# hguo/ftk

Hardware: AMD Instinct MI355X
Metric: space-time simplices/sec (higher is better)
Workload: dtype int64

## Files before the change

ftk_amd/csrc/mask_kernels.hip:

```cpp
#include <atomic>
#include "internal.hpp"
#include "mask_plan.hpp"
#include "sweep_device.hpp"
#include "series_device.hpp"

namespace ftkx {

__device__ inline void red_commit(u64 *red, double mn, double mx, unsigned slot)
{
  for (int o = 32; o > 0; o >>= 1) { mn = fmin(mn, __shfl_down(mn, o)); mx = fmax(mx, __shfl_down(mx, o)); }
  if ((threadIdx.x & 63) == 0) {
    atomicMin(&red[2 * (slot & 63u)], (u64)__double_as_longlong(mn));
    atomicMax(&red[2 * (slot & 63u) + 1], (u64)__double_as_longlong(mx));
  }
}

template <int ND>
__global__ __launch_bounds__(kThreads) void mask_kernel(const Mesh m, const MaskJob *__restrict__ jobs)
{
  const MaskJob job = jobs[blockIdx.y];
  const int P = m.mask_pitch, DH = m.ext_sz[1], DD = (ND == 3) ? m.ext_sz[2] : 1;
  const size_t n = (size_t)P * DH * DD;
  double red_mn = DBL_MAX, red_mx = 0.0;
  for (size_t idx = (size_t)blockIdx.x * kThreads + threadIdx.x; idx < n; idx += (size_t)gridDim.x * kThreads) {
// ... 540 lines not shown
            if (cmask & 0x00ffu) { take(dx0 * fx2); take(dy0 * fy2); }
            if (cmask & 0xff00u) { take(dx1 * fx2); take(dy1 * fy2); }
          }
        }
        if (per_vertex_rule) {
          asm volatile("" ::: "memory");
          const double m0 = max_abs2(dx0 * fx2, dy0 * fy2), m1 = max_abs2(dx1 * fx2, dy1 * fy2);
          bits = (m0 >= tbig ? 0u : (bits & 0x00ffu)) | (m1 >= tbig ? 0u : (bits & 0xff00u));
        }
      } else {
      shift_in_signs<ND>(a0, a1, dx0, dx1, dy0, dy1, dz0, dz1, tneg, tpos);
      if (ND == 2) { a0 = ((a0 & 0xcu) << 1) | (a0 & 3u); a1 = ((a1 & 0xcu) << 1) | (a1 & 3u); }
      bits = guard_and_reduce<ND>(a0, a1, dx0, dx1, dy0, dy1, dz0, dz1, u_int && rok, cmask, per_vertex_rule, tbig, ND == 3 ? 0.5 : 1.0, acc0, acc1, red_mn);
      }
      const unsigned keep = u_int ? xkeep : 0u;
      const unsigned neut = u_dom ? xneutral : 0x3f3fu;
      bits = (bits & keep) | neut;
      if (block4) { bw[r] = rok ? bits : 0x3f3fu; return; }
      bool word_uniform = false;
      if (have_u) {
        int q = (int)((bits & (bits >> 8)) & 0x3fu);
        q &= __builtin_amdgcn_update_dpp(q, q, 0xb1 , 0xf, 0xf, false);
        q &= __builtin_amdgcn_update_dpp(q, q, 0x4e , 0xf, 0xf, false);
        if (rok && u_lane) __builtin_amdgcn_raw_buffer_store_b8((unsigned char)q, rU, ucol, uplane + (unsigned)m.u_pitch * (unsigned)r, 0);
        word_uniform = q != 0;
      }
      if (rok && store_ok && !word_uniform)
        __builtin_amdgcn_raw_buffer_store_b16((unsigned short)bits, rM, mcol, mplane + (unsigned)P * (unsigned)r, 0);
    });
    if constexpr (ND == 2 && RY % 4 == 0 && !REDUCE) if (block4) {
      static_for<RY / 4>([&](auto bc) {
        constexpr int b = decltype(bc)::value;
        const unsigned all = (bw[4 * b] & bw[4 * b + 1]) & (bw[4 * b + 2] & bw[4 * b + 3]);
        int q = (int)((all & (all >> 8)) & 0x3fu);
        q &= __builtin_amdgcn_update_dpp(q, q, 0xb1 , 0xf, 0xf, false);
        q &= __builtin_amdgcn_update_dpp(q, q, 0x4e , 0xf, 0xf, false);
        const bool first_ok = ((row_ok >> (4 * b)) & 1) && k < z1;
        if (first_ok && u_lane) __builtin_amdgcn_raw_buffer_store_b8((unsigned char)q, rU, ucol, (unsigned)m.u_pitch * ((unsigned)(j0 / 4 + b) + (unsigned)((DH + 3) / 4) * (unsigned)k), 0);
        if (q == 0 && store_ok) {
#pragma unroll
          for (int r = 4 * b; r < 4 * b + 4; r ++)
            if (((row_ok >> r) & 1) && k < z1) __builtin_amdgcn_raw_buffer_store_b16((unsigned short)bw[r], rM, mcol, mplane + (unsigned)P * (unsigned)r, 0);
        }
      });
    }
  };

  v2d B[NB][RY + 2];
  double X[NB];
  for (int b = 0; b < NB; b ++) X[b] = 0.0;
  load_plane(B[0], X[0], z0 - 1);
  load_plane(B[1], X[1], z0);
  if (ND == 3) { for (int b = 2; b < 2 + PD; b ++) load_plane(B[b], X[b], z0 + b - 1 < z1 ? z0 + b - 1 : z1); }
  else for (int b = 2; b < NB; b ++) for (int r = 0; r < RY + 2; r ++) B[b][r] = B[1][r];
  for (int k = z0; k < z1; k += NB) {
#pragma unroll
    for (int i = 0; i < NB; i ++)
      step(B[i], B[(i + 1) % NB], B[(i + 2) % NB], B[(i + 2 + PD) % NB], X[(i + 1) % NB], X[(i + 2 + PD) % NB], k + i);
  }
  const unsigned slot = blockIdx.x + blockIdx.y * 7u + blockIdx.z * 13u + (unsigned)wv;
  if constexpr (REDUCE) red_commit(job.red, red_mn, red_mx, slot);
  else if (job.red) {
    const double h = (ND == 3) ? 0.5 : 1.0;
    double mx = fmax((cmask & 0x00ffu) ? acc0 : 0.0, (cmask & 0xff00u) ? acc1 : 0.0) * h;
    if constexpr (LEAN) {
      const double mxx = fmax((cmask & 0x00ffu) ? acc0 : 0.0, (cmask & 0xff00u) ? acc1 : 0.0) * fx2;
      const double mxy = fmax((cmask & 0x00ffu) ? accy0 : 0.0, (cmask & 0xff00u) ? accy1 : 0.0) * fy2;
      mx = max_plain(mxx, mxy);
    }
    red_commit(job.red, red_mn < job.threshold ? red_mn : DBL_MAX, mx, slot);
  }
}

template <int RY>
__global__ __launch_bounds__(256) void mask_rows2_kernel(const Mesh m, const MaskJob *__restrict__ jobs, int groups, int swizzle)
{
  static_assert(RY == 8, "two 8 x 4 blocks per group; the edge register holds 2 RY <= 16 values");
  const int DW = m.ext_sz[0], DH = m.ext_sz[1], P = m.mask_pitch;
  unsigned bx, by, bz;
  remap_block(swizzle, bx, by, bz);
  const MaskJob job = jobs[bz];
  const int lane = threadIdx.x & 63;
  const int wv = __builtin_amdgcn_readfirstlane((int)(threadIdx.x >> 6));
  const int wpb = blockDim.x >> 6;
  const int i0 = (int)bx * 128 + 2 * lane;
  const int jbase = ((int)by * wpb + wv) * RY * groups;
  if (jbase >= DH) return;
  const int jend = jbase + RY * groups < DH ? jbase + RY * groups : DH;
  const unsigned sy = (unsigned)DW * 8u;
  const __amdgpu_buffer_rsrc_t rS = __builtin_amdgcn_make_buffer_rsrc((void *)job.S, 0, (int)(sy * (unsigned)DH), 0x00020000);
  const __amdgpu_buffer_rsrc_t rM = __builtin_amdgcn_make_buffer_rsrc((void *)job.M, 0, (int)((unsigned)P * (unsigned)DH), 0x00020000);
  const __amdgpu_buffer_rsrc_t rU = __builtin_amdgcn_make_buffer_rsrc((void *)job.U, 0, (int)((unsigned)m.u_pitch * (unsigned)DH), 0x00020000);
  const bool have_u = job.U != nullptr;
  const bool block4 = have_u && m.u_rows == 4;
  const double thr = job.threshold;
  const int ic = i0 < DW ? i0 : DW - 2;
  const unsigned cb = (unsigned)ic * 8u;
  const int t0c = (int)bx * 128;
  const int xr = lane < RY ? lane : (lane >= 64 - RY ? lane - (64 - RY) : -1);
  const unsigned xcol8 = (unsigned)(lane < RY ? (t0c > 0 ? t0c - 1 : 0) : (t0c + 128 < DW ? t0c + 128 : DW - 1)) * 8u;
  unsigned xkeep = 0, xneutral = 0;
  for (int c = 0; c < 2; c ++) {
    const int i = i0 + c;
    const bool x_dom = i < DW && i + m.ext_st[0] >= m.dom_lb[0] && i + m.ext_st[0] <= m.dom_ub[0];
    xkeep |= 0x3fu << (8 * c);
    if (!x_dom) xneutral |= 0x3fu << (8 * c);
  }
  const bool in_row = i0 < DW;
  const unsigned mcol = (unsigned)i0, ucol = (unsigned)(i0 >> 3);
  const bool u_lane = (lane & 3) == 0 && in_row;
  double red_mn = DBL_MAX;
  double acc0 = 0.0, acc1 = 0.0, accy0 = 0.0, accy1 = 0.0;
  const unsigned cmask = in_row ? (xkeep & 0x0303u) : 0u;
  const double tbig = job.big;
  const bool per_vertex_rule = job.big < HUGE_VAL;
  const double fx2 = (double)(DW - 1), fy2 = (double)(DH - 1);
  const double tpx = job.tx > 0.0 ? job.tx : exact_threshold(thr, fx2), tpy = job.ty > 0.0 ? job.ty : exact_threshold(thr, fy2);

  struct Rows { unsigned roff[RY + 2]; unsigned row_dom, row_ok, xoff, cbv; int j0; };
  auto setup = [&](Rows &R, int j0) {
    R.j0 = j0;
    const bool live = j0 < jend;
    R.row_dom = 0; R.row_ok = 0;
    for (int r = 0; r < RY + 2; r ++) {
      const int j = j0 + r - 1;
      R.roff[r] = sy * (unsigned)clampi(j, 0, DH - 1);
      if (r >= 1 && r <= RY) {
        if (j < jend) R.row_ok |= 1u << (r - 1);
        if (j + m.ext_st[1] >= m.dom_lb[1] && j + m.ext_st[1] <= m.dom_ub[1]) R.row_dom |= 1u << (r - 1);
      }
    }
    R.cbv = live ? cb : 0xfffffff0u;
    R.xoff = (live && xr >= 0) ? sy * (unsigned)clampi(j0 + xr, 0, DH - 1) + xcol8 : 0xfffffff0u;
  };
  auto load = [&](v2d (&B)[RY + 2], double &X, const Rows &R) {
    for (int r = 0; r < RY + 2; r ++) B[r] = __builtin_bit_cast(v2d, __builtin_amdgcn_raw_buffer_load_b128(rS, R.cbv, R.roff[r], 0));
    X = __builtin_bit_cast(double, __builtin_amdgcn_raw_buffer_load_b64(rS, R.xoff, 0, 0));
  };
  auto step = [&](const v2d (&CU)[RY + 2], const double XC, const Rows &R) {
    const unsigned mplane = (unsigned)P * (unsigned)R.j0, uplane = (unsigned)m.u_pitch * (unsigned)R.j0;
    unsigned bw[RY];
    static_for<RY>([&](auto rc) {
      constexpr int r = decltype(rc)::value;
      const v2d c = CU[r + 1];
      const double xe = edge_for_row<r, RY>(XC);
      const double xm = dpp_lower_or(c.y, xe);
      double xp = dpp_upper_or(c.x, xe);
      if (i0 + 1 == DW - 1) xp = c.y;
      const double dx0 = c.y - xm, dx1 = xp - c.x;
      const double dy0 = CU[r + 2].x - CU[r].x, dy1 = CU[r + 2].y - CU[r].y;
      const bool rok = (R.row_ok >> r) & 1, u_dom = (R.row_dom >> r) & 1;
      unsigned a0 = 0, a1 = 0;
      shift_in_signs2(a0, a1, dx0, dx1, dy0, dy1, -tpx, tpx, -tpy, tpy);
      unsigned bits = a0 | (a1 << 8);
      if (rok) {
        acc0 = max_with_abs(acc0, dx0); acc1 = max_with_abs(acc1, dx1);
        accy0 = max_with_abs(accy0, dy0); accy1 = max_with_abs(accy1, dy1);
        const unsigned u = bits | (bits >> 3);
        if (__builtin_amdgcn_ballot_w64((~u & cmask) != 0u)) {
          auto take = [&](double g) { const double a = fabs(g); red_mn = fmin(red_mn, a == 0.0 ? DBL_MAX : a); };
          if (cmask & 0x00ffu) { take(dx0 * fx2); take(dy0 * fy2); }
          if (cmask & 0xff00u) { take(dx1 * fx2); take(dy1 * fy2); }
        }
      }
      if (per_vertex_rule) {
        asm volatile("" ::: "memory");
        const double m0 = max_abs2(dx0 * fx2, dy0 * fy2), m1 = max_abs2(dx1 * fx2, dy1 * fy2);
        bits = (m0 >= tbig ? 0u : (bits & 0x00ffu)) | (m1 >= tbig ? 0u : (bits & 0xff00u));
      }
      const unsigned neut = u_dom ? xneutral : 0x3f3fu;
      bits = (bits & xkeep) | neut;
      if (block4) { bw[r] = rok ? bits : 0x3f3fu; return; }
      bool word_uniform = false;
      if (have_u) {
        int q = (int)((bits & (bits >> 8)) & 0x3fu);
        q &= __builtin_amdgcn_update_dpp(q, q, 0xb1 , 0xf, 0xf, false);
        q &= __builtin_amdgcn_update_dpp(q, q, 0x4e , 0xf, 0xf, false);
        if (rok && u_lane) __builtin_amdgcn_raw_buffer_store_b8((unsigned char)q, rU, ucol, uplane + (unsigned)m.u_pitch * (unsigned)r, 0);
        word_uniform = q != 0;
      }
      if (rok && in_row && !word_uniform) __builtin_amdgcn_raw_buffer_store_b16((unsigned short)bits, rM, mcol, mplane + (unsigned)P * (unsigned)r, 0);
    });
    if (block4) {
      static_for<RY / 4>([&](auto bc) {
        constexpr int b = decltype(bc)::value;
        const unsigned all = (bw[4 * b] & bw[4 * b + 1]) & (bw[4 * b + 2] & bw[4 * b + 3]);
        int q = (int)((all & (all >> 8)) & 0x3fu);
        q &= __builtin_amdgcn_update_dpp(q, q, 0xb1 , 0xf, 0xf, false);
        q &= __builtin_amdgcn_update_dpp(q, q, 0x4e , 0xf, 0xf, false);
        const bool first_ok = (R.row_ok >> (4 * b)) & 1;
        if (first_ok && u_lane) __builtin_amdgcn_raw_buffer_store_b8((unsigned char)q, rU, ucol, (unsigned)m.u_pitch * (unsigned)(R.j0 / 4 + b), 0);
        if (q == 0 && in_row) {
#pragma unroll
          for (int r = 4 * b; r < 4 * b + 4; r ++)
            if ((R.row_ok >> r) & 1) __builtin_amdgcn_raw_buffer_store_b16((unsigned short)bw[r], rM, mcol, mplane + (unsigned)P * (unsigned)r, 0);
        }
      });
    }
  };

  Rows Ra, Rb;
  v2d A[RY + 2], B[RY + 2];
  double XA, XB;
  setup(Ra, jbase);
  load(A, XA, Ra);
  for (int g = 0; g < groups; g += 2) {
    setup(Rb, jbase + (g + 1) * RY);
    load(B, XB, Rb);
    step(A, XA, Ra);
    setup(Ra, jbase + (g + 2) * RY);
    load(A, XA, Ra);
    if (g + 1 < groups) step(B, XB, Rb);
  }
  if (job.red) {
    const double mxx = fmax((cmask & 0x00ffu) ? acc0 : 0.0, (cmask & 0xff00u) ? acc1 : 0.0) * fx2;
    const double mxy = fmax((cmask & 0x00ffu) ? accy0 : 0.0, (cmask & 0xff00u) ? accy1 : 0.0) * fy2;
    red_commit(job.red, red_mn < job.threshold ? red_mn : DBL_MAX, max_plain(mxx, mxy), blockIdx.x + blockIdx.y * 7u + blockIdx.z * 13u + (unsigned)wv);
  }
}

template <int R> __device__ inline void pack_pair_and(unsigned &T, unsigned bits)
{
  if constexpr (R == 0) asm("v_and_b32_sdwa %0, %1, %1 dst_sel:BYTE_0 dst_unused:UNUSED_PAD src0_sel:BYTE_0 src1_sel:BYTE_1" : "=v"(T) : "v"(bits));
  else if constexpr (R == 1) asm("v_and_b32_sdwa %0, %1, %1 dst_sel:BYTE_1 dst_unused:UNUSED_PRESERVE src0_sel:BYTE_0 src1_sel:BYTE_1" : "+v"(T) : "v"(bits));
  else if constexpr (R == 2) asm("v_and_b32_sdwa %0, %1, %1 dst_sel:BYTE_2 dst_unused:UNUSED_PRESERVE src0_sel:BYTE_0 src1_sel:BYTE_1" : "+v"(T) : "v"(bits));
  else asm("v_and_b32_sdwa %0, %1, %1 dst_sel:BYTE_3 dst_unused:UNUSED_PRESERVE src0_sel:BYTE_0 src1_sel:BYTE_1" : "+v"(T) : "v"(bits));
}
__device__ inline void quad_and(unsigned &T)
{
  asm("s_nop 1\n\t"
      "v_and_b32_dpp %0, %0, %0 quad_perm:[1,0,3,2] row_mask:0xf bank_mask:0xf\n\t"
      "s_nop 1\n\t"
      "v_and_b32_dpp %0, %0, %0 quad_perm:[2,3,0,1] row_mask:0xf bank_mask:0xf"
      : "+v"(T));
}
__device__ inline void row_quads_or(unsigned &x)
{
  asm("s_nop 1\n\t"
      "v_or_b32_dpp %0, %0, %0 row_ror:4 row_mask:0xf bank_mask:0xf\n\t"
      "s_nop 1\n\t"
      "v_or_b32_dpp %0, %0, %0 row_ror:8 row_mask:0xf bank_mask:0xf"
      : "+v"(x));
}
__device__ inline unsigned select_lanes(unsigned a, unsigned b, unsigned long long mask)
{
  unsigned r;
  asm("v_cndmask_b32_e64 %0, %1, %2, %3" : "=v"(r) : "v"(a), "v"(b), "s"(mask));
  return r;
}
template <int R> __device__ inline void byte_nonzero(unsigned long long &mask, unsigned T, unsigned zero)
{
  if constexpr (R == 0) asm volatile("v_cmp_ne_u32_sdwa %0, %1, %2 src0_sel:BYTE_0 src1_sel:DWORD" : "=s"(mask) : "v"(T), "v"(zero));
  else if constexpr (R == 1) asm volatile("v_cmp_ne_u32_sdwa %0, %1, %2 src0_sel:BYTE_1 src1_sel:DWORD" : "=s"(mask) : "v"(T), "v"(zero));
  else if constexpr (R == 2) asm volatile("v_cmp_ne_u32_sdwa %0, %1, %2 src0_sel:BYTE_2 src1_sel:DWORD" : "=s"(mask) : "v"(T), "v"(zero));
  else asm volatile("v_cmp_ne_u32_sdwa %0, %1, %2 src0_sel:BYTE_3 src1_sel:DWORD" : "=s"(mask) : "v"(T), "v"(zero));
}
__device__ inline unsigned out_of_range_where(unsigned off, unsigned long long mask)
{
  unsigned r;
  asm volatile("v_cndmask_b32_e64 %0, %1, -16, %2" : "=v"(r) : "v"(off), "s"(mask));
  return r;
}
template <int I> __device__ inline void lds_read128(v2d &d, unsigned a) { asm volatile("ds_read_b128 %0, %1 offset:%2" : "=v"(d) : "v"(a), "n"(I * 1024)); }
template <int I> __device__ inline void lds_read64(double &d, unsigned a) { asm volatile("ds_read_b64 %0, %1 offset:%2" : "=v"(d) : "v"(a), "n"(I)); }
__device__ inline void lds_tie(v2d &d) { asm volatile("" : "+v"(d)); }
__device__ inline void lds_tie(double &d) { asm volatile("" : "+v"(d)); }
template <int N, int... I> __device__ inline void lds_rows(v2d (&B)[N], unsigned a, std::integer_sequence<int, I...>) { (lds_read128<I>(B[I], a), ...); }
template <int N, int... I> __device__ inline void lds_tie_rows(v2d (&B)[N], std::integer_sequence<int, I...>) { (lds_tie(B[I]), ...); }
template <int RIGHT, int N, int... I> __device__ inline void lds_edges(double (&XL)[N], double (&XR)[N], unsigned a, std::integer_sequence<int, I...>)
{
  (lds_read64<8 * I>(XL[I], a), ...);
  (lds_read64<RIGHT + 8 * I>(XR[I], a), ...);
}
template <int N, int... I> __device__ inline void lds_tie_edges(double (&XL)[N], double (&XR)[N], std::integer_sequence<int, I...>) { ((lds_tie(XL[I]), lds_tie(XR[I])), ...); }

template <int NS, int RY, int S>
__device__ inline void wait_plane_landed(int s)
{
  static_assert((NS - 1) * RY + NS * S < 64 && NS <= 4, "vmcnt is a 6-bit counter; four early steps are spelled out");
#define FTKX_WAIT_VM(N) __builtin_amdgcn_s_waitcnt(((N) & 15) | (7 << 4) | (15 << 8) | (((N) >> 4) << 14))
  if (s >= NS) FTKX_WAIT_VM((NS - 1) * RY + NS * S);
  else if (s == 1) FTKX_WAIT_VM((NS - 1) * RY + S);
  else if (s == 2) FTKX_WAIT_VM((NS - 1) * RY + 2 * S);
  else if (s == 3) FTKX_WAIT_VM((NS - 1) * RY + 3 * S);
  else FTKX_WAIT_VM((NS - 1) * RY);
#undef FTKX_WAIT_VM
}


template <int NS, int CY, int RY, bool TWOB>
__device__ __forceinline__ void march6_body(const Mesh &m, const MaskJob *__restrict__ jobs, int swizzle, int njobs, const ZPlan &plan)
{
#if defined(__HIP_DEVICE_COMPILE__)
  constexpr int ROWS = RY * CY, TROWS = ROWS + 2, NE = NS + 1;
  constexpr bool EDGE2 = ROWS > 16;
  static_assert(ROWS <= 32 && CY >= (EDGE2 ? 4 : 3), "the odd jobs (two halo rows, edge values) go to different wavefronts");
  constexpr unsigned ROWB = 1024u, SLOT = TROWS * ROWB, EDGEB = EDGE2 ? 512u : 256u, ERIGHT = EDGE2 ? 256u : 128u, ERING = NS * SLOT;
  constexpr int DEPTH = TWOB ? NS : NS - 1;
  static_assert(DEPTH >= 1, "at least one plane on its way");
  extern __shared__ __attribute__((aligned(16))) char lds[];
  const int DW = m.ext_sz[0], DH = m.ext_sz[1], DD = m.ext_sz[2], P = m.mask_pitch;
  unsigned bx, by, bz;
  remap_block(swizzle, bx, by, bz);
  const unsigned nj = (unsigned)(njobs < 0 ? -njobs : njobs);
  const unsigned piece = njobs < 0 ? bz % plan.npieces : bz / nj;
  const MaskJob job = jobs[njobs < 0 ? bz / plan.npieces : bz - piece * nj];
  const int z0 = (int)plan.z0[piece];
  const int z1 = z0 + (int)plan.len[piece];
  const int lane = threadIdx.x & 63;
  const int wv = __builtin_amdgcn_readfirstlane((int)(threadIdx.x >> 6));
  const int jb = (int)by * ROWS, t0c = (int)bx * 128;
  if (jb >= DH) return;
  const unsigned sy = (unsigned)DW * 8u, sz = (unsigned)DW * (unsigned)DH * 8u;
  const __amdgpu_buffer_rsrc_t rS = __builtin_amdgcn_make_buffer_rsrc((void *)job.S, 0, (int)(sz * (unsigned)DD), 0x00020000);
  const int nsteps = ((z1 - z0 + 2) / 3) * 3;
  auto slot_of = [&](int q) -> unsigned { return (unsigned)(((q - (z0 - 1)) % NS + NS) % NS) * SLOT; };
  auto edge_of = [&](int q) -> unsigned { return ERING + (unsigned)(((q - (z0 - 1)) % NE + NE) % NE) * EDGEB; };

  const int ip = t0c + 2 * lane;
  const unsigned cb = (unsigned)(ip < DW ? ip : DW - 2) * 8u;
  unsigned eoff = 0xfffffff0u;
  if (wv == 1 || (EDGE2 && wv == 2)) {
    const int e = lane >> 1, row = EDGE2 ? e : (e & 15);
    const bool left = EDGE2 ? wv == 1 : e < 16;
    if (row < ROWS) {
      const int col = left ? (t0c > 0 ? t0c - 1 : 0) : (t0c + 128 < DW ? t0c + 128 : DW - 1);
      eoff = sy * (unsigned)clampi(jb + row, 0, DH - 1) + (unsigned)col * 8u + 4u * (unsigned)(lane & 1);
    }
  }
  unsigned roff[RY];
  for (int r = 0; r < RY; r ++) roff[r] = sy * (unsigned)clampi(jb + wv * RY + r, 0, DH - 1);
  const int xt = wv == 0 ? 0 : TROWS - 1;
  const unsigned xoff = sy * (unsigned)clampi(jb + xt - 1, 0, DH - 1);
  auto issue = [&](int q) {
    const unsigned zo = sz * (unsigned)clampi(q, 0, DD - 1);
    const unsigned base = slot_of(q);
    for (int r = 0; r < RY; r ++) {
      __attribute__((address_space(3))) void *dst = (__attribute__((address_space(3))) void *)(lds + base + (unsigned)(1 + wv * RY + r) * ROWB);
      __builtin_amdgcn_raw_ptr_buffer_load_lds(rS, dst, 16, cb, zo + roff[r], 0, 0);
    }
    if (wv == 0 || wv == CY - 1) {
      __attribute__((address_space(3))) void *dst = (__attribute__((address_space(3))) void *)(lds + base + (unsigned)xt * ROWB);
      __builtin_amdgcn_raw_ptr_buffer_load_lds(rS, dst, 16, cb, zo + xoff, 0, 0);
    } else if (wv == 1 || (EDGE2 && wv == 2)) {
      __attribute__((address_space(3))) void *edst = (__attribute__((address_space(3))) void *)(lds + edge_of(q) + ((EDGE2 && wv == 2) ? ERIGHT : 0u));
      __builtin_amdgcn_raw_ptr_buffer_load_lds(rS, edst, 4, eoff, zo, 0, 0);
    }
  };
#define FTKX_WAIT_VM(N) __builtin_amdgcn_s_waitcnt(((N) & 15) | (7 << 4) | (15 << 8) | (((N) >> 4) << 14))

  const int wy = wv;
  const int i0 = t0c + 2 * lane;
  const __amdgpu_buffer_rsrc_t rM = __builtin_amdgcn_make_buffer_rsrc((void *)job.M, 0, (int)((unsigned)P * (unsigned)DH * (unsigned)DD), 0x00020000);
  const __amdgpu_buffer_rsrc_t rU = __builtin_amdgcn_make_buffer_rsrc((void *)job.U, 0, job.U ? (int)((unsigned)m.u_pitch * (unsigned)DH * (unsigned)DD) : 0, 0x00020000);
  const double thr = job.threshold;
  const double tpos = 2.0 * thr, tneg = -tpos;
  const int j0 = jb + wy * RY;
  unsigned xkeep = 0, xneutral = 0;
  for (int c = 0; c < 2; c ++) {
    const int i = i0 + c;
    const bool x_dom = i < DW && i + m.ext_st[0] >= m.dom_lb[0] && i + m.ext_st[0] <= m.dom_ub[0];
    const bool x_int = i >= 1 && i < DW - 1;
    if (x_int) xkeep |= 0x3fu << (8 * c);
    if (!x_dom) xneutral |= 0x3fu << (8 * c);
  }
  unsigned row_dom = 0, row_int = 0, row_ok = 0;
  for (int r = 0; r < RY; r ++) {
    const int j = j0 + r;
    if (j < DH) row_ok |= 1u << r;
    if (j + m.ext_st[1] >= m.dom_lb[1] && j + m.ext_st[1] <= m.dom_ub[1]) row_dom |= 1u << r;
    if (j >= 1 && j < DH - 1) row_int |= 1u << r;
  }
  const bool in_row = i0 < DW;
  constexpr unsigned OOB = 0xfffffff0u;
  const bool have_u = job.U != nullptr;
  const unsigned mcol = in_row ? (unsigned)i0 : OOB;
  const unsigned ucol = ((lane & 3) == 0 && in_row && have_u) ? (unsigned)(i0 >> 3) : OOB;
  double acc0 = 0.0, acc1 = 0.0, red_mn = DBL_MAX;
  const unsigned cmask = in_row ? (xkeep & 0x0707u) : 0u;
  const double tbig = 2.0 * job.big;
  const bool per_vertex_rule = job.big < HUGE_VAL;
  const unsigned lds0 = (unsigned)(__UINTPTR_TYPE__)(__attribute__((address_space(3))) char *)lds;
  const unsigned lrow = lds0 + (unsigned)(wy * RY) * ROWB + (unsigned)(lane * 16);
  const unsigned eown = lds0 + (unsigned)(wy * RY) * 8u;
  unsigned uoff[RY], moff[RY];
  for (int r = 0; r < RY; r ++) {
    const bool rok = (row_ok >> r) & 1;
    uoff[r] = (rok && ucol != OOB) ? ucol + (unsigned)m.u_pitch * (unsigned)r : OOB;
    moff[r] = (rok && in_row) ? mcol + (unsigned)P * (unsigned)r : OOB;
  }
  const bool wave_interior = (row_ok & row_int & row_dom) == (1u << RY) - 1u;
  const bool batched = RY == 4 && have_u;
  const bool block4 = batched && m.u_rows == 4;
  const bool block16 = batched && CY == 4 && m.u_rows == 16;
  const bool blk = block4 || block16;
  const unsigned a_l = ((unsigned)lane >> 2) & 3u, r_l = (unsigned)lane & 3u, g_l = (unsigned)lane >> 4;
  const unsigned urows = (unsigned)((DH + m.u_rows - 1) / m.u_rows);
  const unsigned uplane_stride = (unsigned)m.u_pitch * urows;
  const unsigned uo4 = (blk ? ((block4 || wy == 0) && r_l == 0 && (row_ok & 1u)) : ((row_ok >> r_l) & 1u)) ? a_l * uplane_stride + (blk ? 0u : r_l * (unsigned)m.u_pitch) + (unsigned)(t0c >> 3) + 4u * g_l : OOB;
  const unsigned psel = (0x0c0c0c0cu & ~(0xffu << (8u * a_l))) | (r_l << (8u * a_l));
  unsigned uacc = 0u;
  const unsigned vzero = 0u;
  const unsigned xch = lds0 + ERING + (unsigned)NE * EDGEB + (unsigned)(lane >> 2) * 4u;
  unsigned t_prev = 0u;
  int k_prev = 0;
  bool pend = false;
  auto finish_prev = [&](unsigned g4) {
    unsigned t = g4 & (g4 >> 16);
    t &= t >> 8;
    const unsigned G = t & 0xffu;
    const unsigned uplane_prev = (unsigned)m.u_pitch * ((unsigned)(j0 / m.u_rows) + urows * (unsigned)k_prev);
    if (wy == 0) {
      const int j = (k_prev - z0) & 3;
      unsigned c = G << (8u * a_l);
      row_quads_or(c);
      uacc = select_lanes(uacc, c, 0x000f000f000f000full << (4 * j));
      if (j == 3 || k_prev == z1 - 1) {
        const unsigned off = j == 3 ? uo4 : (a_l <= (unsigned)j ? uo4 : OOB);
        __builtin_amdgcn_raw_buffer_store_b32(uacc, rU, off, uplane_prev - (unsigned)j * uplane_stride, 0);
      }
    }
    const bool need = G == 0u && t_prev != 0u;
    if (__builtin_amdgcn_ballot_w64(need)) {
      asm volatile("" ::: "memory");
      const unsigned v = t_prev | (t_prev << 8);
      const unsigned mp = (unsigned)P * ((unsigned)j0 + (unsigned)DH * (unsigned)k_prev);
      static_for<RY>([&](auto rc) { constexpr int r = decltype(rc)::value; __builtin_amdgcn_raw_buffer_store_b16((unsigned short)v, rM, need ? moff[r] : OOB, mp, 0); });
    }
    pend = false;
  };

  auto take_plane = [&](v2d (&B)[RY + 2], int q) { lds_rows(B, lrow + slot_of(q), std::make_integer_sequence<int, RY + 2>{}); };
  auto landed = [&](v2d (&B)[RY + 2]) {
    asm volatile("s_waitcnt lgkmcnt(0)" ::: "memory");
    lds_tie_rows(B, std::make_integer_sequence<int, RY + 2>{});
  };

  auto step = [&](const v2d (&PR)[RY + 2], const v2d (&CU)[RY + 2], v2d (&NX)[RY + 2], int k) {
    if (batched) wait_plane_landed<DEPTH, RY, RY>(k - z0);
    else wait_plane_landed<DEPTH, RY, 2 * RY>(k - z0);
    if (block16) asm volatile("s_waitcnt lgkmcnt(0)" ::: "memory");
    __builtin_amdgcn_s_barrier();
    const bool live = k < z1;
    if constexpr (!TWOB) { const int q = k + NS; issue(q < z1 ? q : z1); }
    double XL[RY], XR[RY];
    const bool fin = block16 && pend;
    unsigned g4 = 0u;
    if (fin) asm volatile("ds_read_b32 %0, %1" : "=v"(g4) : "v"(xch + (unsigned)(k_prev & 1) * 64u));
    if (live) {
      take_plane(NX, k + 1 < z1 ? k + 1 : z1);
      lds_edges<(int)ERIGHT>(XL, XR, eown + edge_of(k), std::make_integer_sequence<int, RY>{});
      landed(NX);
      lds_tie_edges(XL, XR, std::make_integer_sequence<int, RY>{});
    } else if (fin) asm volatile("s_waitcnt lgkmcnt(0)" ::: "memory");
    if (fin) { asm volatile("" : "+v"(g4)); finish_prev(g4); }
    if constexpr (TWOB) {
      __builtin_amdgcn_s_barrier();
      const int q = k + 1 + NS; issue(q < z1 ? q : z1);
    }
    if (!live) return;
    const bool z_dom = k + m.ext_st[2] >= m.dom_lb[2] && k + m.ext_st[2] <= m.dom_ub[2];
    const bool z_int = k >= 1 && k < DD - 1;
    const unsigned mplane = (unsigned)P * ((unsigned)j0 + (unsigned)DH * (unsigned)k);
    const unsigned uplane = (unsigned)m.u_pitch * ((unsigned)(j0 / m.u_rows) + urows * (unsigned)k);
    unsigned bw[RY];
    unsigned raw_and = 0xffffffffu;
    auto rows = [&](auto interior_c, auto rule_c) {
      constexpr bool INTERIOR = decltype(interior_c)::value, RULE = decltype(rule_c)::value;
      static_for<RY>([&](auto rc) {
        constexpr int r = decltype(rc)::value;
        const v2d c = CU[r + 1];
        const double xm = dpp_lower_or(c.y, XL[r]), xp = dpp_upper_or(c.x, XR[r]);
        const double dx0 = c.y - xm, dx1 = xp - c.x;
        const double dy0 = CU[r + 2].x - CU[r].x, dy1 = CU[r + 2].y - CU[r].y;
        const double dz0 = NX[r + 1].x - PR[r + 1].x, dz1 = NX[r + 1].y - PR[r + 1].y;
        unsigned a0 = 0, a1 = 0;
        shift_in_signs<3>(a0, a1, dx0, dx1, dy0, dy1, dz0, dz1, tneg, tpos);
        double m0 = max_abs2(dx0, dy0), m1 = max_abs2(dx1, dy1);
        m0 = max_with_abs(m0, dz0); m1 = max_with_abs(m1, dz1);
        unsigned bits = a0 | (a1 << 8);
        const bool u_int = INTERIOR || (((row_int >> r) & 1) && z_int), u_dom = INTERIOR || (((row_dom >> r) & 1) && z_dom);
        if (INTERIOR || (u_int && ((row_ok >> r) & 1))) {
          acc0 = max_plain(acc0, m0); acc1 = max_plain(acc1, m1);
          raw_and &= bits;
        }
        if constexpr (RULE) bits = (m0 >= tbig ? 0u : (bits & 0x00ffu)) | (m1 >= tbig ? 0u : (bits & 0xff00u));
        if constexpr (INTERIOR) bits = (bits & xkeep) | xneutral;
        else bits = (bits & (u_int ? xkeep : 0u)) | (u_dom ? xneutral : 0x3f3fu);
        bw[r] = bits;
      });
    };
    const bool interior = z_int && z_dom && wave_interior;
    if (interior) { if (per_vertex_rule) rows(std::true_type{}, std::true_type{}); else rows(std::true_type{}, std::false_type{}); }
    else { if (per_vertex_rule) rows(std::false_type{}, std::true_type{}); else rows(std::false_type{}, std::false_type{}); }
    {
      const unsigned u = raw_and | (raw_and >> 3);
      if (__builtin_amdgcn_ballot_w64((~u & cmask) != 0u)) {
        static_for<RY>([&](auto rc) {
          constexpr int r = decltype(rc)::value;
          if (((row_int >> r) & 1) && z_int && ((row_ok >> r) & 1)) {
            const v2d c = CU[r + 1];
            const double xm = dpp_lower_or(c.y, XL[r]), xp = dpp_upper_or(c.x, XR[r]);
            auto take = [&](double d) { const double a = fabs(0.5 * d); red_mn = fmin(red_mn, a == 0.0 ? DBL_MAX : a); };
            if (cmask & 0x00ffu) { take(c.y - xm); take(CU[r + 2].x - CU[r].x); take(NX[r + 1].x - PR[r + 1].x); }
            if (cmask & 0xff00u) { take(xp - c.x); take(CU[r + 2].y - CU[r].y); take(NX[r + 1].y - PR[r + 1].y); }
          }
        });
      }
    }
    unsigned T[(RY + 3) / 4];
    unsigned long long wu[RY];
    unsigned mo[RY];
    if (blk) {
      if constexpr (RY == 4) {
        unsigned all = bw[0] & bw[1];
        all &= bw[2] & bw[3];
        pack_pair_and<0>(T[0], all);
        quad_and(T[0]);
        byte_nonzero<0>(wu[0], T[0], vzero);
        asm volatile("s_nop 1");
        static_for<RY>([&](auto rc) { constexpr int r = decltype(rc)::value; mo[r] = out_of_range_where(moff[r], wu[0]); });
      }
    } else {
      static_for<RY>([&](auto rc) { constexpr int r = decltype(rc)::value; pack_pair_and<r % 4>(T[r / 4], bw[r]); });
      static_for<(RY + 3) / 4>([&](auto gc) { quad_and(T[decltype(gc)::value]); });
      if (!have_u) static_for<(RY + 3) / 4>([&](auto gc) { T[decltype(gc)::value] = 0u; });
      static_for<RY>([&](auto rc) { constexpr int r = decltype(rc)::value; byte_nonzero<r % 4>(wu[r], T[r / 4], vzero); });
      if constexpr (RY < 3) asm volatile("s_nop 1");
      static_for<RY>([&](auto rc) { constexpr int r = decltype(rc)::value; mo[r] = out_of_range_where(moff[r], wu[r]); });
    }
    if (block16) {
      asm volatile("ds_write_b8 %0, %1" :: "v"(xch + (unsigned)(k & 1) * 64u + (unsigned)wy), "v"(T[0]) : "memory");
      t_prev = T[0]; k_prev = k; pend = true;
      static_for<RY>([&](auto rc) { constexpr int r = decltype(rc)::value; __builtin_amdgcn_raw_buffer_store_b16((unsigned short)bw[r], rM, mo[r], mplane, 0); });
      return;
    }
    if (batched) {
      const int j = (k - z0) & 3;
      unsigned c = block4 ? (T[0] << (8u * a_l)) : __builtin_amdgcn_perm(0u, T[0], psel);
      row_quads_or(c);
      uacc = select_lanes(uacc, c, 0x000f000f000f000full << (4 * j));
      if (j == 3 || k == z1 - 1) {
        const unsigned off = j == 3 ? uo4 : (a_l <= (unsigned)j ? uo4 : OOB);
        __builtin_amdgcn_raw_buffer_store_b32(uacc, rU, off, uplane - (unsigned)j * uplane_stride, 0);
      }
      static_for<RY>([&](auto rc) { constexpr int r = decltype(rc)::value; __builtin_amdgcn_raw_buffer_store_b16((unsigned short)bw[r], rM, mo[r], mplane, 0); });
      return;
    }
    static_for<RY>([&](auto rc) {
      constexpr int r = decltype(rc)::value;
      __builtin_amdgcn_raw_buffer_store_b8((unsigned char)(T[r / 4] >> (8 * (r % 4))), rU, uoff[r], uplane, 0);
      __builtin_amdgcn_raw_buffer_store_b16((unsigned short)bw[r], rM, mo[r], mplane, 0);
    });
  };

  v2d B[3][RY + 2];
  issue(z0 - 1); issue(z0);
  FTKX_WAIT_VM(0);
  __builtin_amdgcn_s_barrier();
  take_plane(B[0], z0 - 1);
  take_plane(B[1], z0);
  landed(B[0]); landed(B[1]);
  __builtin_amdgcn_s_barrier();
  for (int q = z0 + 1; q <= z0 + DEPTH; q ++) issue(q < z1 ? q : z1);
  for (int s = 0; s < nsteps; s += 3) {
    step(B[0], B[1], B[2], z0 + s);
    step(B[1], B[2], B[0], z0 + s + 1);
    step(B[2], B[0], B[1], z0 + s + 2);
  }
  if (block16 && pend) {
    asm volatile("s_waitcnt lgkmcnt(0)" ::: "memory");
    __builtin_amdgcn_s_barrier();
    unsigned g4;
    asm volatile("ds_read_b32 %0, %1\n\ts_waitcnt lgkmcnt(0)" : "=v"(g4) : "v"(xch + (unsigned)(k_prev & 1) * 64u) : "memory");
    finish_prev(g4);
  }
  FTKX_WAIT_VM(0);
#undef FTKX_WAIT_VM
  if (job.red) {
    const double mx = fmax((cmask & 0x00ffu) ? acc0 : 0.0, (cmask & 0xff00u) ? acc1 : 0.0) * 0.5;
    red_commit(job.red, red_mn < job.threshold ? red_mn : DBL_MAX, mx, blockIdx.x + blockIdx.y * 7u + blockIdx.z * 13u + (unsigned)wv);
  }
#endif
}

template <int NS, int CY, int RY, bool TWOB>
__global__ __launch_bounds__(64 * CY) void mask_march6_kernel(const Mesh m, const MaskJob *__restrict__ jobs, int swizzle, int njobs, const ZPlan plan)
{
  march6_body<NS, CY, RY, TWOB>(m, jobs, swizzle, njobs, plan);
}
template <int ND>
__global__ __launch_bounds__(kThreads) void resolution_scalar_kernel(const Mesh m, const double *__restrict__ S, u64 *out)
{
  u64 mn = 0x7fefffffffffffffull, mx = 0ull;
  const int DW = m.ext_sz[0], DH = m.ext_sz[1], DD = (ND == 3) ? m.ext_sz[2] : 1;
  const size_t n = (size_t)DW * DH * DD;
  for (size_t idx = (size_t)blockIdx.x * kThreads + threadIdx.x; idx < n; idx += (size_t)gridDim.x * kThreads) {
    const int i = (int)(idx % DW), j = (int)((idx / DW) % DH), k = (int)(idx / ((size_t)DW * DH));
    double g[ND];
    gradient_at<ND>(m, S, i, j, k, g);
    for (int c = 0; c < ND; c ++) {
      const double a = fabs(g[c]);
      const u64 bits = (u64)__double_as_longlong(a);
      if (a != 0.0 && bits < 0x7ff0000000000000ull) { mn = bits < mn ? bits : mn; mx = bits > mx ? bits : mx; }
    }
  }
  for (int o = 32; o > 0; o >>= 1) {
    const u64 omn = __shfl_down(mn, o), omx = __shfl_down(mx, o);
    mn = omn < mn ? omn : mn; mx = omx > mx ? omx : mx;
// ... 83 lines not shown
```

ftk_amd/csrc/mask_plan.hpp:

```cpp
#pragma once
#include <algorithm>
#include <cstdlib>
#include <cstring>
#include <vector>

namespace ftkx {

struct ZPlan {
  unsigned npieces;
  unsigned z0[47], len[47];
};

constexpr long kHookUnset = -0x7fffffffL;
struct MaskHooks {
  long swizzle = kHookUnset, yg = kHookUnset, zchunk = kHookUnset, lmin = kHookUnset, lcap = kHookUnset, order = kHookUnset, rows = kHookUnset, lean = kHookUnset;
  long u_rows = 0;
};
inline long hook_or(long v, long dflt) { return v == kHookUnset ? dflt : v; }

inline MaskHooks parse_mask_hooks(const char *plan, const char *u_rows)
{
  MaskHooks h;
  const struct { const char *name; long MaskHooks::*knob; } knobs[] = {{"swizzle", &MaskHooks::swizzle}, {"yg", &MaskHooks::yg}, {"zchunk", &MaskHooks::zchunk},
    {"lmin", &MaskHooks::lmin}, {"lcap", &MaskHooks::lcap}, {"order", &MaskHooks::order}, {"rows", &MaskHooks::rows}, {"lean", &MaskHooks::lean}};
  for (const char *p = plan ? plan : ""; *p;) {
    while (*p == ',' || *p == ' ') p ++;
    for (const auto &k : knobs) {
      const size_t n = strlen(k.name);
      if (!strncmp(p, k.name, n) && p[n] == '=' && h.*k.knob == kHookUnset) h.*k.knob = atol(p + n + 1);
    }
    while (*p && *p != ',') p ++;
  }
  if (u_rows) h.u_rows = atoi(u_rows);
  return h;
}
inline MaskHooks read_mask_hooks() { return parse_mask_hooks(getenv("FTKX_MASK_PLAN"), getenv("FTKX_U_ROWS")); }

struct MaskShape { int nd, scalar_mode, ext_sz[3], mask_pitch; };

enum MaskFamily { MASK_MARCH6 = 0 , MASK_MARCH4 = 1 , MASK_ROWS2 = 2 ,
                  MASK_REDUCE = 3 , MASK_VEC2 = 4 ,
                  MASK_VEC = 5 , MASK_GENERIC = 6, MASK_FAMILIES = 7 };
constexpr unsigned kMaskThreads = 256;

struct MaskPlan {
  MaskFamily family;
  const char *name;
  bool march2;
  bool has_summary;
  int u_rows;
  unsigned grid[3], block, lds_bytes;
  int swizzle, zchunk, groups, njobs;
  ZPlan z;
};

inline MaskPlan plan_masks(const MaskShape &s, const MaskHooks &h, int njobs, bool reduce)
{
  MaskPlan p = MaskPlan();
  const int DW = s.ext_sz[0], DH = s.ext_sz[1], DD = s.nd == 3 ? s.ext_sz[2] : 1;
  const size_t nrows = (size_t)DH * (size_t)DD;
  p.march2 = s.scalar_mode && (DW % 2) == 0 && DW >= 2 && (size_t)DW * nrows * 8 < (1ull << 32);
  const bool vec_fast = !s.scalar_mode && DW >= 8 && (DW % 8) == 0;
  const bool vec_lean = vec_fast && DW >= 256 && hook_or(h.lean, 1) != 0 && (size_t)DW * nrows * 8 * (size_t)s.nd < (1ull << 31) && (size_t)s.mask_pitch * nrows < (1ull << 31);
  p.has_summary = h.u_rows >= 0 && (s.scalar_mode ? p.march2 && (DW % 8) == 0 : vec_fast);
  if (!p.has_summary || h.u_rows == 1) p.u_rows = 1;
  else if (!s.scalar_mode) p.u_rows = vec_lean ? 4 : 1;
  else if (s.nd == 3) p.u_rows = h.u_rows == 4 ? 4 : 16;
  else p.u_rows = 4;
  p.njobs = njobs;
  p.block = kMaskThreads;
  p.grid[1] = p.grid[2] = 1;
  if (p.march2) {
    int swizzle = 8;
    if (s.nd == 2) swizzle |= 16;
    swizzle = (int)hook_or(h.swizzle, swizzle);
    int zchunk = 32;
    const bool zforced = hook_or(h.zchunk, 0) > 0;
    if (zforced) zchunk = (int)h.zchunk;
    auto yg_of = [&](int dflt) { const long v = h.yg == kHookUnset ? dflt : h.yg > 0 ? h.yg : 1; return (int)(v > 255 ? 255 : v); };
    auto grouped = [](int sw, int yg) { return (sw & 0xff) | (yg << 8); };
    p.grid[0] = (unsigned)((DW + 127) / 128);
    if (s.nd == 3 && !reduce) {
      const int yg_want = yg_of(16);
      int lmin = 6, lcap = 24;
      if (hook_or(h.lmin, 0) >= 1) lmin = (int)h.lmin;
      if (hook_or(h.lcap, 0) >= 1) lcap = (int)h.lcap;
      if (lcap < lmin) lcap = lmin;
      std::vector<int> lens;
      int rem = DD;
      if (zforced) while (rem > 0) { const int l = rem < zchunk ? rem : zchunk; lens.push_back(l); rem -= l; }
      while (rem > 0) {
        int l = (rem + 1) / 2;
        if (l > lcap) l = lcap;
        if (l < lmin) l = lmin;
        if (l >= 3) l -= l % 3;
        if (l > rem || rem - l < (lmin + 1) / 2) l = rem;
        lens.push_back(l); rem -= l;
      }
      while (lens.size() > 47) { const int l = lens.back(); lens.pop_back(); lens.back() += l; }
      std::stable_sort(lens.begin(), lens.end(), [](int a, int b) { return a > b; });
      p.z.npieces = (unsigned)lens.size();
      int z = 0;
      for (size_t i = 0; i < lens.size(); i ++) { p.z.z0[i] = (unsigned)z; p.z.len[i] = (unsigned)lens[i]; z += lens[i]; }
      constexpr int NS6 = 2, CY6 = 4, RY6 = 4, rows = CY6 * RY6;
      p.family = MASK_MARCH6; p.name = "ftkx::mask_march6_kernel<2, 4, 4, false>";
      p.block = 64u * CY6;
      p.grid[1] = (unsigned)((DH + rows - 1) / rows); p.grid[2] = p.z.npieces * (unsigned)njobs;
      p.swizzle = swizzle;
      if (swizzle & 8) { int yg = yg_want; if (yg > (int)p.grid[1]) yg = (int)p.grid[1]; p.grid[1] = (p.grid[1] + (unsigned)yg - 1) / (unsigned)yg * (unsigned)yg; p.swizzle = grouped(swizzle, yg); }
      p.lds_bytes = (unsigned)NS6 * (unsigned)(rows + 2) * 1024u + (unsigned)(NS6 + 1) * 256u + 128u;
      bool slice_major = (size_t)p.grid[0] * ((DH + rows - 1) / rows) * p.z.npieces >= 768;
      if (h.order != kHookUnset) slice_major = h.order == 0;
      if (slice_major) p.njobs = -njobs;
      return p;
    }
    const int RY = (s.nd == 3) ? 4 : 8, wpb = 4;
    p.block = (unsigned)(64 * wpb);
    int groups = 0;
    if (s.nd == 2 && !reduce) {
      groups = (int)hook_or(h.rows, (DW >= 4096 && DH >= 512) ? 4 : 0);
      if (groups > 64) groups = 64;
    }
    const int wg_rows = groups >= 1 ? wpb * RY * groups : wpb * RY;
    p.grid[1] = (unsigned)((DH + wg_rows - 1) / wg_rows);
    if (swizzle & 8) {
      int yg = yg_of(4);
      while (yg > 1 && p.grid[1] % (unsigned)yg) yg --;
      swizzle = grouped(swizzle, yg);
    }
    p.swizzle = swizzle;
    if (groups >= 1) { p.family = MASK_ROWS2; p.name = "ftkx::mask_rows2_kernel<8>"; p.groups = groups; p.grid[2] = (unsigned)njobs; return p; }
    const int nzc = s.nd == 3 ? (DD + zchunk - 1) / zchunk : 1;
    p.grid[2] = (unsigned)(nzc * njobs);
    p.zchunk = zchunk;
    p.family = reduce ? MASK_REDUCE : MASK_MARCH4;
    p.name = !reduce ? "ftkx::mask_march4_kernel<2, false, 1, 8>" : s.nd == 2 ? "ftkx::mask_march4_kernel<2, true, 1, 8>" : "ftkx::mask_march4_kernel<3, true, 1, 4>";
    return p;
  }
  p.grid[1] = (unsigned)njobs;
  if (vec_fast) {
    const size_t groups = (size_t)(DW / 4) * nrows;
    size_t bx = (groups + kMaskThreads - 1) / kMaskThreads;
    if (bx > 2048) bx = 2048;
    while (bx > 256 && bx * kMaskThreads * 4 > groups) bx /= 2;
    if (p.u_rows == 4) {
      const size_t units = (size_t)((DW / 4 + 63) / 64) * ((DH + 3) / 4) * (size_t)DD;
      bx = (units + 7) / 8;
      if (bx > 2048) bx = 2048;
    }
    p.grid[0] = (unsigned)bx;
    p.family = p.u_rows == 4 ? MASK_VEC2 : MASK_VEC;
    p.name = p.u_rows == 4 ? (s.nd == 2 ? "ftkx::mask_vec2_kernel<2>" : "ftkx::mask_vec2_kernel<3>") : (s.nd == 2 ? "ftkx::mask_vec_kernel<2>" : "ftkx::mask_vec_kernel<3>");
    return p;
  }
  const size_t n = (size_t)s.mask_pitch * nrows;
  size_t bx = (n + kMaskThreads - 1) / kMaskThreads;
  if (bx > 4096) bx = 4096;
  p.grid[0] = (unsigned)bx;
  p.family = MASK_GENERIC; p.name = s.nd == 2 ? "ftkx::mask_kernel<2>" : "ftkx::mask_kernel<3>";
  return p;
}

}
```

Measured before the change: 45130 billion.

## Group jobs into slice-major batches when decoding march6 block indices

Adds an sgroup field to the z-plan and a shared decode routine that, in slice-major order, interleaves z-pieces across small groups of jobs instead of across all jobs. The group size is picked so that a group's blocks fit within a concurrency budget of about 768 blocks and align with the y-group swizzle. The aim is to keep neighbouring z-pieces of the same few jobs resident together, improving cache locality for halo planes and balancing load. It adds integer divisions to the per-block index decode and a new tuning knob.

```diff
diff --git a/ftk_amd/csrc/mask_kernels.hip b/ftk_amd/csrc/mask_kernels.hip
--- a/ftk_amd/csrc/mask_kernels.hip
+++ b/ftk_amd/csrc/mask_kernels.hip
@@ -866,9 +866,9 @@
   const int DW = m.ext_sz[0], DH = m.ext_sz[1], DD = m.ext_sz[2], P = m.mask_pitch;
   unsigned bx, by, bz;
   remap_block(swizzle, bx, by, bz);
-  const unsigned nj = (unsigned)(njobs < 0 ? -njobs : njobs);
-  const unsigned piece = njobs < 0 ? bz % plan.npieces : bz / nj;
-  const MaskJob job = jobs[njobs < 0 ? bz / plan.npieces : bz - piece * nj];
+  const ZWhere at = zplan_decode(plan, njobs, bz);
+  const unsigned piece = at.piece;
+  const MaskJob job = jobs[at.job];
   const int z0 = (int)plan.z0[piece];
   const int z1 = z0 + (int)plan.len[piece];
   const int lane = threadIdx.x & 63;
diff --git a/ftk_amd/csrc/mask_plan.hpp b/ftk_amd/csrc/mask_plan.hpp
--- a/ftk_amd/csrc/mask_plan.hpp
+++ b/ftk_amd/csrc/mask_plan.hpp
@@ -9,11 +9,33 @@
 struct ZPlan {
   unsigned npieces;
   unsigned z0[47], len[47];
+  unsigned sgroup;
 };
+
+#if defined(__HIPCC__)
+#define FTKX_PLAN_HD __host__ __device__
+#else
+#define FTKX_PLAN_HD
+#endif
+
+struct ZWhere { unsigned job, piece; };
+FTKX_PLAN_HD inline ZWhere zplan_decode(const ZPlan &plan, int njobs, unsigned bz)
+{
+  ZWhere w;
+  if (njobs >= 0) { w.piece = bz / (unsigned)njobs; w.job = bz - w.piece * (unsigned)njobs; return w; }
+  const unsigned nj = (unsigned)-njobs, t = bz / plan.npieces;
+  if (plan.sgroup == 0) { w.piece = bz - t * plan.npieces; w.job = t; return w; }
+  const unsigned ngroups = (nj + plan.sgroup - 1) / plan.sgroup, small = nj / ngroups, extra = nj - small * ngroups, head = extra * (small + 1);
+  const unsigned size = t < head ? small + 1 : small;
+  const unsigned first = t < head ? t / size * size : head + (t - head) / size * size;
+  const unsigned r = bz - first * plan.npieces;
+  w.piece = r / size; w.job = first + (r - w.piece * size);
+  return w;
+}
 
 constexpr long kHookUnset = -0x7fffffffL;
 struct MaskHooks {
-  long swizzle = kHookUnset, yg = kHookUnset, zchunk = kHookUnset, lmin = kHookUnset, lcap = kHookUnset, order = kHookUnset, rows = kHookUnset, lean = kHookUnset;
+  long swizzle = kHookUnset, yg = kHookUnset, zchunk = kHookUnset, lmin = kHookUnset, lcap = kHookUnset, order = kHookUnset, sgroup = kHookUnset, rows = kHookUnset, lean = kHookUnset;
   long u_rows = 0;
 };
 inline long hook_or(long v, long dflt) { return v == kHookUnset ? dflt : v; }
@@ -22,7 +44,7 @@
 {
   MaskHooks h;
   const struct { const char *name; long MaskHooks::*knob; } knobs[] = {{"swizzle", &MaskHooks::swizzle}, {"yg", &MaskHooks::yg}, {"zchunk", &MaskHooks::zchunk},
-    {"lmin", &MaskHooks::lmin}, {"lcap", &MaskHooks::lcap}, {"order", &MaskHooks::order}, {"rows", &MaskHooks::rows}, {"lean", &MaskHooks::lean}};
+    {"lmin", &MaskHooks::lmin}, {"lcap", &MaskHooks::lcap}, {"order", &MaskHooks::order}, {"sgroup", &MaskHooks::sgroup}, {"rows", &MaskHooks::rows}, {"lean", &MaskHooks::lean}};
   for (const char *p = plan ? plan : ""; *p;) {
     while (*p == ',' || *p == ' ') p ++;
     for (const auto &k : knobs) {
@@ -110,8 +132,18 @@
       if (swizzle & 8) { int yg = yg_want; if (yg > (int)p.grid[1]) yg = (int)p.grid[1]; p.grid[1] = (p.grid[1] + (unsigned)yg - 1) / (unsigned)yg * (unsigned)yg; p.swizzle = grouped(swizzle, yg); }
       p.lds_bytes = (unsigned)NS6 * (unsigned)(rows + 2) * 1024u + (unsigned)(NS6 + 1) * 256u + 128u;
       bool slice_major = (size_t)p.grid[0] * ((DH + rows - 1) / rows) * p.z.npieces >= 768;
-      if (h.order != kHookUnset) slice_major = h.order == 0;
+      bool grouped_slices = slice_major && njobs > 1;
+      if (h.order != kHookUnset) { slice_major = h.order == 0 || h.order == 2; grouped_slices = h.order == 2; }
       if (slice_major) p.njobs = -njobs;
+      if (grouped_slices) {
+        const unsigned per_piece = p.grid[0] * p.grid[1], pgroups = (p.swizzle & 8) ? p.grid[1] / (((unsigned)p.swizzle >> 8) & 0xffu) : 0;
+        unsigned fits = 768 / per_piece, sg = 0;
+        if (fits > (unsigned)njobs) fits = (unsigned)njobs;
+        for (unsigned c = fits; c >= 1 && !sg; c --) if (pgroups && (c * pgroups) % 8 == 0) sg = c;
+        if (!sg) sg = fits >= 1 ? fits : 1;
+        if (h.sgroup != kHookUnset) sg = (unsigned)(h.sgroup < 1 ? 1 : h.sgroup > njobs ? njobs : h.sgroup);
+        p.z.sgroup = sg;
+      }
       return p;
     }
     const int RY = (s.nd == 3) ? 4 : 8, wpb = 4;
```

After: 46410 billion (median of 6 runs). 2.8% higher.
